# shijun18/H-DenseFormer

Hardware: AMD Instinct MI355X
Metric: train samples/sec on 4x128^3 volumes (higher is better)
Workload: dtype bf16

## Files before the change

h-denseformer_amd/csrc/transformer_chain.hip:

```cpp
#include <mutex>

#include "tf_tok.h"

namespace {

using namespace tftok;

constexpr int CT = 512;
constexpr int KVC = 128;
constexpr int KVP = 68;
constexpr int LDQ = 100;
constexpr int SYNC_LINE = 32;
constexpr int FR_KA = 0;
constexpr int FR_VA = 64;
constexpr int FR_QA = 128;
constexpr int FR_KB = 192;
constexpr int FR_QB = 232;
constexpr int FR_W = 288;
constexpr int XG_GA = 0;
constexpr int XG_GB = 64;
constexpr int XG_W = 128;
constexpr float LOG2E = 1.4426950408889634f, LN2 = 0.6931471805599453f;
constexpr int ATRIP = 16;
typedef float f2 __attribute__((ext_vector_type(2)));
// ... 186 lines not shown
}
__device__ __forceinline__ float4 ld16_sc1(__amdgpu_buffer_rsrc_t r, uint32_t byte_off) {
  return __builtin_bit_cast(float4, __builtin_amdgcn_raw_buffer_load_b128(r, byte_off, 0, 16));
}
__device__ __forceinline__ void chain_arrive(unsigned* cnt, bool storing = true) {
  if (storing) asm volatile("s_waitcnt vmcnt(0)" ::: "memory");
  __syncthreads();
  if (threadIdx.x == 0) __hip_atomic_fetch_add(cnt, 1u, __ATOMIC_RELAXED, __HIP_MEMORY_SCOPE_AGENT);
}
using ChainCtl = TfChainCtl;
__device__ __forceinline__ void chain_wait(unsigned* cnt, unsigned target, unsigned* tmo, const ChainCtl& c, bool& dead) {
  if (threadIdx.x == 0 && !dead) {
    const uint64_t t_start = __builtin_amdgcn_s_memrealtime();
    unsigned spins = 0;
    while (__hip_atomic_load(cnt, __ATOMIC_RELAXED, __HIP_MEMORY_SCOPE_AGENT) < target) {
      __builtin_amdgcn_s_sleep(2);
      if ((++spins & 31u) == 0u && __hip_atomic_load(tmo, __ATOMIC_RELAXED, __HIP_MEMORY_SCOPE_AGENT) != 0u) {
        dead = true;
        break;
      }
      if (__builtin_amdgcn_s_memrealtime() - t_start > (uint64_t)c.ticks) {
        __hip_atomic_store(tmo, 1u + blockIdx.x, __ATOMIC_RELAXED, __HIP_MEMORY_SCOPE_AGENT);
        if (c.host_flag) __hip_atomic_store(c.host_flag, 1u + blockIdx.x, __ATOMIC_RELAXED, __HIP_MEMORY_SCOPE_SYSTEM);
        dead = true;
        break;
      }
    }
  }
  __builtin_amdgcn_fence(__ATOMIC_ACQUIRE, "wavefront");
  __syncthreads();
}
__device__ __forceinline__ bool chain_any_dead(bool dead, unsigned* word) {
  __syncthreads();
  if (threadIdx.x == 0) *word = dead ? 1u : 0u;
  __syncthreads();
  return *word != 0u;
}

#ifdef CHAIN_DBG_STAMPS
#define CHAIN_STAMP(k)                                                                                   \
  do {                                                                                                   \
    if (threadIdx.x == 0)                                                                                \
      reinterpret_cast<uint64_t*>(a.sync + (1 << 18))[((size_t)blockIdx.x * 32 + L) * 16 + (k)] = __builtin_amdgcn_s_memrealtime(); \
  } while (0)
#define CHAIN_STAMPB(k)                                                                                  \
  do {                                                                                                   \
    if (threadIdx.x == 0)                                                                                \
      reinterpret_cast<uint64_t*>(a.sync + (1 << 18) + (1 << 17))[((size_t)blockIdx.x * 32 + (L + 1)) * 16 + (k)] = __builtin_amdgcn_s_memrealtime(); \
  } while (0)
#else
#define CHAIN_STAMP(k) ((void)0)
#define CHAIN_STAMPB(k) ((void)0)
#endif

struct ChainFwd {
  TfDims d;
  ChainW cw;
  const float* params;
  const float4* wpack;
  int dtype;
  float* F0;
  float* save;
  void* attnall;
  unsigned* sync;
  TfChainCtl ctl;
  float* frag;
  int nb, ntile, nseq;
  int64_t rows;
};

template <bool TRAIN>
__global__ __launch_bounds__(CT) void tf_chain_fwd_kernel(ChainFwd a) {
  HDF_CHAIN_PRIO();
  extern __shared__ __attribute__((aligned(16))) float sm[];
  const TfDims& d = a.d;
  const int DM = d.DM, DMF = d.DMF, ldF = DMF + 4, N = d.N, BN = d.B * N;
  float* s_F = sm;
  float* s_x = s_F + TT * ldF;
  float* s_h = s_x + TT * LD32;
  float* s_z = s_h + TT * LD32;
  float* s_red = s_z + TT * LD64;
  float* s_ob = s_red + 2 * 16 * 16;
  float* s_q = s_ob + TT * LD32;
  float* s_kv = s_q + TT * LDQ;
  const int tid = threadIdx.x, lane = tid & 63, wave8 = tid >> 6, wave = wave8 & 3, col = lane & 15, g = lane >> 4;
  const bool cw = tid < 256;
  const int seq = blockIdx.x % a.nseq, tile = blockIdx.x / a.nseq;
  const int m = seq / d.B, bsm = seq - m * d.B;
  const int n0 = tile * TT, nvalid = min(TT, N - n0);
  const int t0k = bsm * N + n0;
  const int64_t mo = (int64_t)m * d.mstride, rb = (int64_t)m * BN;
  const DropF dr{TRAIN ? 1 : 0, d.seed, d.thresh24, d.keep_scale};
  auto tok = [&](int row) { return t0k + min(row, nvalid - 1); };
  float* pm = const_cast<float*>(a.params);
  unsigned* cnt = a.sync + seq * SYNC_LINE;
  unsigned* tmo = a.sync + a.nseq * SYNC_LINE;
  bool dead = false;
  const int nl = a.nb * 4;
  const int cw_col = 16 * (wave & 1) + col, c4w = 16 * wave + col;

  WFrag<2> f_wo{}, f_w1{};
  WFrag<4> f_w2{};
  WFrag<11> f_w0{};
  WFrag<2> f_q0{}, f_q1{};
  float p_bout = 0.f, p_b1 = 0.f, p_b2 = 0.f, p_b0 = 0.f;
  LnP ln2{}, ln1{};
// ... 374 lines not shown
        const float inv = 1.f / l;
        const float4 o = make_float4(a01.x * inv, a01.y * inv, a23.x * inv, a23.y * inv);
        *reinterpret_cast<float4*>(s_ob + col * LD32 + head * 4) = o;
        const float lsv = __builtin_fmaf(mx, LN2, __logf(l));
        if (col < nvalid) {
          float* ob = sv + a.rows * 128;
          float* lse = sv + a.rows * 160;
          const int64_t R = rb + t0 + col;
          *reinterpret_cast<float4*>(ob + R * 32 + head * 4) = o;
          lse[R * 8 + head] = lsv;
        }
        if (a.frag)
          a.frag[(int64_t)nl * a.nseq * a.ntile * 8 * FR_W + (((int64_t)L * a.nseq + seq) * 8 + head) * (a.ntile * TT) + n0 + col] =
              col < nvalid ? -lsv * LOG2E : -INFINITY;
      }
      CHAIN_STAMP(7);
    }
  }
  if (chain_any_dead(dead, reinterpret_cast<unsigned*>(s_red))) {
    const float qnan = __builtin_nanf("");
    for (int i = tid; i < nvalid * DM; i += CT) {
      const int row = i / DM, c = i - row * DM;
      const int64_t ai = ((int64_t)bsm * N + n0 + row) * ((int64_t)d.M * DM) + (int64_t)m * DM + c;
      if (a.dtype == HDF_BF16)
        ST<bf16_t>::st(reinterpret_cast<bf16_t*>(a.attnall) + ai, qnan);
      else if (a.dtype == HDF_F16)
        ST<f16_t>::st(reinterpret_cast<f16_t*>(a.attnall) + ai, qnan);
      else
        reinterpret_cast<float*>(a.attnall)[ai] = qnan;
    }
  }
}

struct ChainBwd {
  TfDims d;
  ChainW cw;
  const float* params;
  float* grads;
  const float* F0;
  const float* save;
  float* dF;
  const void* d_attnall;
  const float4* wpack;
  float* tape;
  float* otape;
  float* xchg;
  const float* frag;
  unsigned* sync;
  TfChainCtl ctl;
  int nb, ntile, nseq, dtype;
  int64_t rows;
};

constexpr int QC = 64;
constexpr int QP = 84;
constexpr int XW = 40;

template <int LP>
struct ChainLp;
template <>
struct ChainLp<1> {
  static __device__ __forceinline__ uint16_t one(float v) { return f2bf(v); }
  static __device__ __forceinline__ u32x2 four(float a, float b, float c, float d) { return u32x2{pack_bf2(a, b), pack_bf2(c, d)}; }
  static __device__ __forceinline__ f32x4 mma(const u32x2& a, const u32x2& b, const f32x4& c) {
    return __builtin_amdgcn_mfma_f32_16x16x16bf16_1k(__builtin_bit_cast(s16x4, a), __builtin_bit_cast(s16x4, b), c, 0, 0, 0);
  }
};
typedef __attribute__((ext_vector_type(4))) _Float16 chain_f16x4;
template <>
struct ChainLp<2> {
  static __device__ __forceinline__ uint16_t one(float v) { return f2h(v); }
  static __device__ __forceinline__ u32x2 four(float a, float b, float c, float d) { return u32x2{pack_h2(a, b), pack_h2(c, d)}; }
  static __device__ __forceinline__ f32x4 mma(const u32x2& a, const u32x2& b, const f32x4& c) {
    return __builtin_amdgcn_mfma_f32_16x16x16f16(__builtin_bit_cast(chain_f16x4, a), __builtin_bit_cast(chain_f16x4, b), c, 0, 0, 0);
  }
};

__device__ __forceinline__ f32x4 chain_mfma4(float a, float b, const f32x4& c) {
  return __builtin_amdgcn_mfma_f32_16x16x4f32(a, b, c, 0, 0, 0);
}

template <bool TRAIN, int LP>
__global__ __launch_bounds__(CT) void tf_chain_bwd_kernel(ChainBwd a) {
  HDF_CHAIN_PRIO();
  extern __shared__ __attribute__((aligned(16))) float sm[];
  const TfDims& d = a.d;
  const int DM = d.DM, DMF = d.DMF, ldF = DMF + 4, ldD = DM + 4, N = d.N, BN = d.B * N;
  float* s_F = sm;
  float* s_dF = s_F + TT * ldF;
  float* s_do = s_dF + TT * ldF;
  float* s_dq = s_do + TT * ldD;
  float* s_a = s_dq + TT * 100;
  float* s_b = s_a + TT * LD32;
  float* s_c = s_b + TT * LD32;
  float* s_e = s_c + TT * LD32;
  float* s_dg = s_e + TT * LD32;
  float* s_gx = s_dg + TT * LD32;
  float* s_dO = s_gx + TT * LD32;
  float* s_f = s_dO + TT * LD32;
  float* s_dz = s_f + TT * LD64;
  float* s_red = s_dz + TT * LD64;
  float* s_dl = s_red + 2 * 16 * 16;
  float* s_at = s_dl + TT * 8;
  constexpr int AT_IMG = QC * QP, AT_T = 8 * QC, AT_U = 8 * 5 * QC / 2;
  constexpr int AT_BUF = AT_IMG + 2 * AT_T + 2 * AT_U;
  const int tid = threadIdx.x, lane = tid & 63, wave8 = tid >> 6, wave = wave8 & 3, col0 = lane & 15, g0 = lane >> 4;
  const bool cw = tid < 256;
  const int lrow0 = (tid >> 4) & 15, lc0 = (tid & 15) * 2;
  const int seq = blockIdx.x % a.nseq, tile = blockIdx.x / a.nseq;
  const int m = seq / d.B, bsm = seq - m * d.B;
  const int n0 = tile * TT, nvalid = min(TT, N - n0);
  const int t0k = bsm * N + n0;
  const int64_t mo = (int64_t)m * d.mstride, rb = (int64_t)m * BN;
  const int64_t trows = a.rows;
  const DropF dr{TRAIN ? 1 : 0, d.seed, d.thresh24, d.keep_scale};
  float* pm = const_cast<float*>(a.params);
  unsigned* cnt = a.sync + seq * SYNC_LINE;
  unsigned* tmo = a.sync + a.nseq * SYNC_LINE;
  bool dead = false;
  const int nl = a.nb * 4;
  float r_acc0 = 0.f, r_acc1 = 0.f;
  const int htid = tid - 256;

  for (int L = nl - 1; L >= -1; L--) {
    const bool PREB = L + 1 < nl, POSTB = L >= 0, OUTB = POSTB && (L & 3) == 3;
    const int Lq = L + 1, bq = Lq >> 2, lq = Lq & 3;
    const int bp = L >> 2, lp = L & 3, bo = bp;
    int t0 = t0k;
    asm volatile("" : "+s"(t0));
    int col = col0, g = g0, lrow = lrow0, lc = lc0;
    asm volatile("" : "+v"(col), "+v"(g), "+v"(lrow), "+v"(lc));
    auto tok = [&](int row) { return t0 + min(row, nvalid - 1); };
    auto tape_h = [&](float* tape, int col0, const float* sT, int lds_ld, int width) __attribute__((always_inline)) {
      const int w4 = width >> 2;
      float* seg = tape + trows * col0 + (rb + t0) * width;
      for (int i = htid; i < TT * w4; i += 256) {
        const int row = i / w4, c4 = (i - row * w4) * 4;
        if (row < nvalid) *reinterpret_cast<float4*>(seg + i * 4) = *reinterpret_cast<const float4*>(sT + row * lds_ld + c4);
      }
    };
    auto colsum_h = [&](float* gb, int width, const float* sv, int ld, int tbase) __attribute__((always_inline)) {
      const int c = htid - tbase;
      if (c >= 0 && c < width) {
        float acc = 0.f;
#pragma unroll
        for (int r = 0; r < TT; r++) acc += sv[r * ld + c];
        atomicAdd(gb + c, acc);
      }
    };
    const bool lok = lrow < nvalid;
    const int64_t lr = (rb + tok(lrow)) * 32 + lc;
    const int Kq = PREB ? DM + 32 * lq : 0;
    CFrag<12> c_q{};
    CFrag<8> c_w0[6]{};
    WFrag<2> f_w1{};
    CFrag<8> c_w2{}, c_w1{};
    CFrag<4> c_wo{};
    LnP ln1{}, ln2{};
    float p_b1 = 0.f, r_h[2][2] = {{0.f, 0.f}, {0.f, 0.f}}, r_ob[2] = {0.f, 0.f}, r_h0[2] = {0.f, 0.f};
    TfLayerP gq{}, gp{};
    if (PREB) {
      float* w0 = chain_w0(a.cw, pm, bq, lq) + mo;
      float* rest = w0 + 32 * Kq;
      float* gw0 = chain_w0(a.cw, a.grads, bq, lq) + mo;
      float* grest = gw0 + 32 * Kq;
      gq.b0 = grest + CO_B0, gq.ln1g = grest + CO_LN1G, gq.ln1b = grest + CO_LN1B;
      if (cw) {
        const float4* slot = a.wpack + ((int64_t)m * nl + Lq) * (CH_SLOT * 64);
        cpload(c_q, slot, CB_Q + 3 * wave);
#pragma unroll
        for (int j = 0; j < 6; j++) cpload(c_w0[j], slot, CB_W0 + 2 * min(wave + 4 * j, (Kq >> 4) - 1));
        ln1 = ln_load(rest + CO_LN1G, rest + CO_LN1B);
        const float* h0 = a.save + (int64_t)Lq * a.rows * 232;
        r_h0[0] = h0[lr], r_h0[1] = h0[lr + 1];
      }
    }
    if (POSTB) {
      float* w0 = chain_w0(a.cw, pm, bp, lp) + mo;
      float* rest = w0 + 32 * (DM + 32 * lp);
      float* grest = chain_w0(a.cw, a.grads, bp, lp) + mo + 32 * (DM + 32 * lp);
      gp.bout = grest + CO_BOUT, gp.ln2g = grest + CO_LN2G, gp.ln2b = grest + CO_LN2B, gp.b1 = grest + CO_B1, gp.b2 = grest + CO_B2;
      if (cw) {
        const float4* slot = a.wpack + ((int64_t)m * nl + L) * (CH_SLOT * 64);
        pload(f_w1, slot, CH_W1 + 2 * wave, 2);
// ... 133 lines not shown
        }
        {
          f32x4 acc = zero4();
          cmma_stream_p(acc, oslot, OB_B + 16 * wave, s_do, ldD, DM >> 2);
          const int c = 16 * wave + col;
#pragma unroll
          for (int r = 0; r < 4; r++) s_dz[(4 * g + r) * LD64 + c] = acc[r] * mk[r] * gelu_grad_f(zr[r]);
        }
      }
      __syncthreads();
      if (!cw) {
        tape_h(otape, 0, s_do, ldD, DM);
        tape_h(otape, DM, s_f, LD64, 64);
        tape_h(otape, DM + 64, s_dz, LD64, 64);
        for (int c0 = 0; c0 < DM; c0 += 128) colsum_h(go.bb + mo + c0, min(128, DM - c0), s_do + c0, ldD, 0);
        colsum_h(go.ba + mo, 64, s_dz, LD64, 128);
      } else {
        for (int nn = 16 * wave; nn < DMF; nn += 64) {
          f32x4 acc = zero4();
          cmma_stream_p(acc, oslot, OA_B + 4 * (nn >> 4), s_dz, LD64, 16);
          const int c = nn + col;
#pragma unroll
          for (int r = 0; r < 4; r++) {
            const int row = 4 * g + r;
            s_dF[row * ldF + c] = acc[r];
            if (c >= DMF - 32) s_dg[row * LD32 + c - (DMF - 32)] = row < nvalid ? acc[r] : 0.f;
          }
        }
      }
      __syncthreads();
    }

    CHAIN_STAMPB(3);
    {
      float* tape_p = a.tape + (int64_t)L * a.rows * TF_TAPE_W;
      const uint32_t site0 = hdf_site_id(m, bp, lp, 0);
      const int t = t0 + lrow;
      const bool ok = lok;
      float dcur0 = 0.f, dcur1 = 0.f;
      if (cw) dcur0 = s_dg[lrow * LD32 + lc], dcur1 = s_dg[lrow * LD32 + lc + 1];
      float dres0 = 0.f, dres1 = 0.f;
#pragma unroll
      for (int pass = 1; pass >= 0; pass--) {
        __syncthreads();
        float rs = 0.f;
        if (cw) {
          s_a[lrow * LD32 + lc] = r_h[pass][0];
          s_a[lrow * LD32 + lc + 1] = r_h[pass][1];
          rs = ln32_keep(s_a, s_b, s_c, ln2);
          s_dg[lrow * LD32 + lc] = ok ? dcur0 * dr.mask(site0 + 2 + 2 * pass, (uint32_t)t * 32 + lc) : 0.f;
          s_dg[lrow * LD32 + lc + 1] = ok ? dcur1 * dr.mask(site0 + 2 + 2 * pass, (uint32_t)t * 32 + lc + 1) : 0.f;
        }
        __syncthreads();
        if (pass == 1) CHAIN_STAMPB(9);
        if (cw) {
          f32x4 accz = zero4(), accd = zero4();
          wmma(accz, f_w1, s_b, LD32, 8, 0, 2);
          cmma(accd, c_w2, s_dg, LD32, 8, 0, 8);
          const int c = 16 * wave + col;
          const float b1 = p_b1;
#pragma unroll
          for (int r = 0; r < 4; r++) {
            const int row = 4 * g + r, tt = t0 + row;
            const float z = accz[r] + b1, mkv = dr.mask(site0 + 1 + 2 * pass, (uint32_t)tt * 64 + c);
            s_f[row * LD64 + c] = row < nvalid ? gelu_f(z) * mkv : 0.f;
            s_dz[row * LD64 + c] = row < nvalid ? accd[r] * mkv * gelu_grad_f(z) : 0.f;
          }
        }
        __syncthreads();
        if (pass == 1) CHAIN_STAMPB(10);
        f32x4 accu = zero4();
        if (!cw) {
          const int c0 = pass ? TF_T_P1 : TF_T_P0;
          tape_h(tape_p, c0, s_dg, LD32, 32);
          tape_h(tape_p, c0 + 32, s_f, LD64, 64);
          tape_h(tape_p, c0 + 96, s_dz, LD64, 64);
          tape_h(tape_p, c0 + 160, s_b, LD32, 32);
          colsum_h(gp.b2, 32, s_dg, LD32, 0);
          colsum_h(gp.b1, 64, s_dz, LD64, 64);
        } else {
          cmma(accu, c_w1, s_dz, LD64, 16, 8 * (wave >> 1), 8);
          if (wave >= 2) {
#pragma unroll
            for (int r = 0; r < 4; r++) s_red[((wave & 1) * 16 + 4 * g + r) * 16 + col] = accu[r];
          }
        }
        __syncthreads();
        if (pass == 1) CHAIN_STAMPB(11);
        if (cw && wave < 2) {
#pragma unroll
          for (int r = 0; r < 4; r++)
            s_e[(4 * g + r) * LD32 + 16 * wave + col] = accu[r] + s_red[(wave * 16 + 4 * g + r) * 16 + col];
        }
        __syncthreads();
        if (pass == 1) CHAIN_STAMPB(12);
        float dh0v = 0.f, dh1v = 0.f;
        if (cw) {
          ln32_bwd(s_e, s_c, s_gx, rs, ln2, dh0v, dh1v);
          dh0v = ok ? dh0v : 0.f, dh1v = ok ? dh1v : 0.f;
        }
        __syncthreads();
        if (pass == 1) CHAIN_STAMPB(13);
        if (!cw) {
          colsum_h(gp.ln2g, 32, s_gx, LD32, 0);
          colsum_h(gp.ln2b, 32, s_e, LD32, 64);
        }
        if (pass == 1) {
          dcur0 = dh0v, dcur1 = dh1v;
          dres0 = dh0v, dres1 = dh1v;
        } else {
          dres0 += dh0v, dres1 += dh1v;
        }
      }
      __syncthreads();
      if (cw) {
        s_dg[lrow * LD32 + lc] = ok ? dres0 * dr.mask(site0 + 0, (uint32_t)t * 32 + lc) : 0.f;
        s_dg[lrow * LD32 + lc + 1] = ok ? dres1 * dr.mask(site0 + 0, (uint32_t)t * 32 + lc + 1) : 0.f;
        s_b[lrow * LD32 + lc] = r_ob[0];
        s_b[lrow * LD32 + lc + 1] = r_ob[1];
        r_acc0 = dres0, r_acc1 = dres1;
      }
      __syncthreads();
      CHAIN_STAMPB(14);
      f32x4 acco = zero4();
      if (!cw) {
        tape_h(tape_p, TF_T_DGO, s_dg, LD32, 32);
        colsum_h(gp.bout, 32, s_dg, LD32, 0);
      } else {
        cmma(acco, c_wo, s_dg, LD32, 8, 4 * (wave >> 1), 4);
        if (wave >= 2) {
#pragma unroll
          for (int r = 0; r < 4; r++) s_red[((wave & 1) * 16 + 4 * g + r) * 16 + col] = acco[r];
        }
      }
      __syncthreads();
      if (cw && wave < 2) {
#pragma unroll
        for (int r = 0; r < 4; r++)
          s_dO[(4 * g + r) * LD32 + 16 * wave + col] = acco[r] + s_red[(wave * 16 + 4 * g + r) * 16 + col];
      }
      __syncthreads();
      CHAIN_STAMPB(15);
      if (tid < TT * 8) {
        const int row = tid >> 3, h = tid & 7;
        s_dl[row * 8 + h] = tf_dot4(*reinterpret_cast<const float4*>(s_dO + row * LD32 + 4 * h),
                                    *reinterpret_cast<const float4*>(s_b + row * LD32 + 4 * h));
      }
      __syncthreads();
    }

    CHAIN_STAMPB(4);
    const int par = L & 1;
    float* xbase = a.xchg + ((int64_t)par * a.rows + rb + (int64_t)bsm * N) * XW;
    const __amdgpu_buffer_rsrc_t rx = chain_rsrc(xbase);
    float* xgseq = a.xchg + ((int64_t)par * a.nseq + seq) * a.ntile * 8 * XG_W;
    if (LP) {
      constexpr int L1 = LP ? LP : 1;
      float* s_rec = s_f;
      {
        const int hd = wave8;
        float* rec = s_rec + hd * XG_W;
        const bool vrow = col < nvalid;
        rec[XG_GA + lane] = vrow ? s_dO[col * LD32 + hd * 4 + g] : 0.f;
        if (lane < 20) {
          const int c = lane >> 2, gg = lane & 3;
          float gv[4] = {0.f, 0.f, 0.f, 0.f};
          if (c < 4) {
#pragma unroll
            for (int e = 0; e < 4; e++) gv[e] = 4 * gg + e < nvalid ? s_dO[(4 * gg + e) * LD32 + hd * 4 + c] : 0.f;
          }
          reinterpret_cast<u32x2*>(rec + XG_GB)[lane] = ChainLp<L1>::four(gv[0], gv[1], gv[2], gv[3]);
        }
        if (lane < 16) rec[XG_GB + 40 + lane] = lane < nvalid ? -s_dl[lane * 8 + hd] : 0.f;
      }
      __syncthreads();
      if (tid < 8 * 26) {
        const int hd = tid / 26, pc = tid - hd * 26;
        const __amdgpu_buffer_rsrc_t rr = chain_rsrc(xgseq + (int64_t)tile * 8 * XG_W);
        st16_sc1(rr, (uint32_t)((hd * XG_W + 4 * pc) * 4), *reinterpret_cast<const float4*>(s_rec + hd * XG_W + 4 * pc));
      } else if (tid < 8 * 26 + 32) {
        const int i = tid - 8 * 26, hd = i >> 2, pc = i & 3;
        const __amdgpu_buffer_rsrc_t rr = chain_rsrc(a.xchg + (int64_t)2 * a.nseq * a.ntile * 8 * XG_W +
                                                     ((int64_t)par * a.nseq + seq) * 8 * (a.ntile * TT));
        st16_sc1(rr, (uint32_t)((hd * (a.ntile * TT) + n0 + 4 * pc) * 4),
                 *reinterpret_cast<const float4*>(s_rec + hd * XG_W + XG_GB + 40 + 4 * pc));
      }
    } else if (tid < TT * 10) {
      const int row = tid / 10, c4 = (tid - row * 10) * 4;
      if (row < nvalid) {
        const float4 v = c4 < 32 ? *reinterpret_cast<const float4*>(s_dO + row * LD32 + c4)
                                 : *reinterpret_cast<const float4*>(s_dl + row * 8 + (c4 - 32));
        st16_sc1(rx, (uint32_t)(((n0 + row) * XW + c4) * 4), v);
      }
    }
    const int head = __builtin_amdgcn_readfirstlane(wave8);
    const float* sv = a.save + (int64_t)L * a.rows * 232;
    const float* qkvL = sv + a.rows * 32 + (rb + (int64_t)bsm * N) * 96;
    const float* lseL = sv + a.rows * 160 + (rb + (int64_t)bsm * N) * 8;
    const int rown = n0 + min(col, nvalid - 1);
    const float own_q = qkvL[(int64_t)rown * 96 + head * 4 + g];
    const float own_k = qkvL[(int64_t)rown * 96 + 32 + head * 4 + g];
    const float own_v = qkvL[(int64_t)rown * 96 + 64 + head * 4 + g];
    const float own_lse = lseL[(int64_t)rown * 8 + head];
    constexpr int PD = 8, NLS = 4;
    const int NPq = attn_rows(N);
    const float* fr = nullptr;
    const int cb = min(col, 4) * 4 + g;
    float ka[PD], va[PD];
    u32x2 kb[PD];
    float4 r_ls[NLS];
    auto ldk = [&](int b, int i) __attribute__((always_inline)) {
      const float* r = fr + (int64_t)min(b, a.ntile - 1) * 8 * FR_W;
      ka[i] = r[FR_KA + lane], va[i] = r[FR_VA + lane];
      kb[i] = reinterpret_cast<const u32x2*>(r + FR_KB)[cb];
    };
    if constexpr (LP != 0) {
      fr = a.frag + ((int64_t)L * a.nseq + seq) * a.ntile * 8 * FR_W + (int64_t)head * FR_W;
      const float* lsrow = a.frag + (int64_t)nl * a.nseq * a.ntile * 8 * FR_W + (((int64_t)L * a.nseq + seq) * 8 + head) * NPq;
#pragma unroll
      for (int i = 0; i < PD; i++) ldk(i, i);
#pragma unroll
      for (int k = 0; k < NLS; k++) r_ls[k] = *reinterpret_cast<const float4*>(lsrow + min((k * 64 + lane) * 4, NPq - 4));
    }
    chain_arrive(cnt, cw);
    CHAIN_STAMPB(5);
    CHAIN_STAMPB(6);

    if constexpr (LP != 0) {
      const int NP = NPq, nblk = a.ntile;
      const float* xg = xgseq + (int64_t)head * XG_W;
      float* s_ls = s_at + head * 2 * NP;
      float* s_dlq = s_ls + NP;
      const __amdgpu_buffer_rsrc_t rdl = chain_rsrc(a.xchg + (int64_t)2 * a.nseq * a.ntile * 8 * XG_W +
                                                    (((int64_t)par * a.nseq + seq) * 8 + head) * NP);
      {
        const float delta = s_dl[col * 8 + head];
        const float ls = own_lse * LOG2E;
        const float bqv = own_q * (0.5f * LOG2E);
        const float bg = s_dO[col * LD32 + head * 4 + g];
        const f32x4 nl4 = {-ls, -ls, -ls, -ls}, nd4 = {-delta, -delta, -delta, -delta};
        f32x4 acc = {0.f, 0.f, 0.f, 0.f};
        auto step = [&](int i, int j0, auto masked) __attribute__((always_inline)) {
          const f32x4 cs = chain_mfma4(ka[i], bqv, nl4), ct = chain_mfma4(va[i], bg, nd4);
          float ds[4];
#pragma unroll
          for (int u = 0; u < 4; u++) {
            ds[u] = __builtin_amdgcn_exp2f(cs[u]) * ct[u];
            if (decltype(masked)::value) ds[u] = (j0 + 4 * g + u < N) ? ds[u] : 0.f;
          }
          acc = ChainLp<LP>::mma(ChainLp<LP>::four(ds[0], ds[1], ds[2], ds[3]), kb[i], acc);
        };
        const int nfullb = N / ATRIP;
        int bb = 0;
        for (; bb + PD <= nfullb; bb += PD) {
#pragma unroll
          for (int i = 0; i < PD; i++) {
            step(i, 0, std::false_type{});
            ldk(bb + i + PD, i);
          }
        }
        for (int i = 0; bb < nblk; bb++, i++) {
#pragma unroll
          for (int k = 0; k < PD; k++)
            if (k == i) {
              if ((bb + 1) * ATRIP <= N)
                step(k, 0, std::false_type{});
              else
                step(k, bb * ATRIP, std::true_type{});
            }
        }
#pragma unroll
        for (int r = 0; r < 4; r++)
          if (col < 4) s_dq[(4 * g + r) * 100 + head * 4 + col] = (4 * g + r < nvalid) ? 0.5f * acc[r] : 0.f;
      }
      chain_wait(cnt, (unsigned)(a.ntile * (nl - L)), tmo, a.ctl, dead);
      {
        float4 r_dl[NLS];
#pragma unroll
        for (int k = 0; k < NLS; k++) r_dl[k] = ld16_sc1(rdl, (uint32_t)(min((k * 64 + lane) * 4, NP - 4) * 4));
#pragma unroll
        for (int k = 0; k < NLS; k++) {
          const int i4 = (k * 64 + lane) * 4;
          if (i4 < NP) {
            *reinterpret_cast<float4*>(s_ls + i4) = r_ls[k];
            *reinterpret_cast<float4*>(s_dlq + i4) = r_dl[k];
          }
        }
      }
      CHAIN_STAMPB(7);
      {
        const float bk = own_k, bv = own_v;
        const float* tl = s_ls + 4 * g;
        const float* td = s_dlq + 4 * g;
        float qa[PD], ga[PD];
        u32x2 qb[PD], gb[PD];
        auto ld = [&](int b, int i) __attribute__((always_inline)) {
          const int bc = min(b, nblk - 1);
          const float* r = fr + (int64_t)bc * 8 * FR_W;
          const float* x = xg + (int64_t)bc * 8 * XG_W;
          qa[i] = r[FR_QA + lane];
          qb[i] = reinterpret_cast<const u32x2*>(r + FR_QB)[cb];
          ga[i] = __hip_atomic_load(x + XG_GA + lane, __ATOMIC_RELAXED, __HIP_MEMORY_SCOPE_AGENT);
          const unsigned long long w = __hip_atomic_load(reinterpret_cast<const unsigned long long*>(x + XG_GB) + cb,
                                                         __ATOMIC_RELAXED, __HIP_MEMORY_SCOPE_AGENT);
          gb[i] = u32x2{(uint32_t)w, (uint32_t)(w >> 32)};
        };
#pragma unroll
        for (int i = 0; i < PD; i++) ld(i, i);
        f32x4 dk = {0.f, 0.f, 0.f, 0.f}, dv = {0.f, 0.f, 0.f, 0.f};
        auto step = [&](int i, int b) __attribute__((always_inline)) {
          const f32x4 l4 = *reinterpret_cast<const f32x4*>(tl + b * ATRIP), d4 = *reinterpret_cast<const f32x4*>(td + b * ATRIP);
          const f32x4 cs = chain_mfma4(qa[i], bk, l4), ct = chain_mfma4(ga[i], bv, d4);
          const float p0 = __builtin_amdgcn_exp2f(cs[0]), p1 = __builtin_amdgcn_exp2f(cs[1]);
          const float p2 = __builtin_amdgcn_exp2f(cs[2]), p3 = __builtin_amdgcn_exp2f(cs[3]);
          dv = ChainLp<LP>::mma(ChainLp<LP>::four(p0, p1, p2, p3), gb[i], dv);
          dk = ChainLp<LP>::mma(ChainLp<LP>::four(p0 * ct[0], p1 * ct[1], p2 * ct[2], p3 * ct[3]), qb[i], dk);
        };
        int bb = 0;
        for (; bb + PD <= nblk; bb += PD) {
#pragma unroll
          for (int i = 0; i < PD; i++) {
            step(i, bb + i);
            ld(bb + i + PD, i);
          }
        }
        for (int i = 0; bb < nblk; bb++, i++) {
#pragma unroll
// ... 29 lines not shown
          const float z = c * QC + srow < N ? 1.f : 0.f;
          float* img = s_at + (c & 1) * AT_BUF;
          const float4 kk = make_float4(pk.x * z, pk.y * z, pk.z * z, pk.w * z);
          *reinterpret_cast<float4*>(img + srow * KVP + 4 * spart) = kk;
          *reinterpret_cast<float4*>(img + srow * KVP + 32 + 4 * spart) = make_float4(pv.x * z, pv.y * z, pv.z * z, pv.w * z);
          if (LP) {
            uint16_t* kt = reinterpret_cast<uint16_t*>(img + AT_IMG + 2 * AT_T) + spart * 5 * QC;
            constexpr int L1 = LP ? LP : 1;
            kt[0 * QC + srow] = ChainLp<L1>::one(kk.x), kt[1 * QC + srow] = ChainLp<L1>::one(kk.y);
            kt[2 * QC + srow] = ChainLp<L1>::one(kk.z), kt[3 * QC + srow] = ChainLp<L1>::one(kk.w);
            kt[4 * QC + srow] = 0;
          }
        };
        stage_load(0);
        stage_store(0);
        __syncthreads();
        f32x4 acc = {0.f, 0.f, 0.f, 0.f};
        f2 d01 = {0.f, 0.f}, d23 = {0.f, 0.f};
        const f32x4 nl4 = {-ls, -ls, -ls, -ls}, nd4 = {-delta, -delta, -delta, -delta}, z4 = {0.f, 0.f, 0.f, 0.f};
        for (int c = 0; c < nchunk; c++) {
          if (c + 1 < nchunk) stage_load(c + 1);
          const float* img = s_at + (c & 1) * AT_BUF;
          const uint16_t* kt = reinterpret_cast<const uint16_t*>(img + AT_IMG + 2 * AT_T) + head * 5 * QC + min(col, 4) * QC + 4 * g;
          const int jbase = c * QC, ntrip = min(QC, NP - jbase) / ATRIP;
          for (int k = 0; k < ntrip; k++) {
            const int jj = k * ATRIP, j0 = jbase + jj;
            const float ka = img[(jj + col) * KVP + head * 4 + g], va = img[(jj + col) * KVP + 32 + head * 4 + g];
            if (LP) {
              constexpr int L1 = LP ? LP : 1;
              const f32x4 cs = chain_mfma4(ka, bqv, nl4), ct = chain_mfma4(va, bg, nd4);
              const u32x2 kb = *reinterpret_cast<const u32x2*>(kt + jj);
              float ds[4];
#pragma unroll
              for (int u = 0; u < 4; u++) {
                ds[u] = __builtin_amdgcn_exp2f(cs[u]) * ct[u];
                if (j0 + ATRIP > N) ds[u] = (j0 + 4 * g + u < N) ? ds[u] : 0.f;
              }
              acc = ChainLp<L1>::mma(ChainLp<L1>::four(ds[0], ds[1], ds[2], ds[3]), kb, acc);
            } else {
              const f32x4 s4 = chain_mfma4(ka, bqv, z4), t4 = chain_mfma4(va, bg, z4);
#pragma unroll
              for (int u = 0; u < 4; u++) {
                const float4 kr = *reinterpret_cast<const float4*>(img + (jj + 4 * g + u) * KVP + head * 4);
                float pr = __builtin_amdgcn_exp2f(s4[u] - ls);
                if (j0 + ATRIP > N) pr = (j0 + 4 * g + u < N) ? pr : 0.f;
                const float dsv = pr * (t4[u] - delta);
                const f2 dd = {dsv, dsv};
                d01 = __builtin_elementwise_fma(dd, lo2(kr), d01);
                d23 = __builtin_elementwise_fma(dd, hi2(kr), d23);
              }
            }
          }
          if (c + 1 < nchunk) stage_store(c + 1);
          __syncthreads();
        }
        if (LP) {
#pragma unroll
          for (int r = 0; r < 4; r++)
            if (col < 4) s_dq[(4 * g + r) * 100 + head * 4 + col] = (4 * g + r < nvalid) ? 0.5f * acc[r] : 0.f;
        } else {
#pragma unroll
          for (int off = 16; off < 64; off <<= 1) {
            d01.x += __shfl_xor(d01.x, off, 64), d01.y += __shfl_xor(d01.y, off, 64);
            d23.x += __shfl_xor(d23.x, off, 64), d23.y += __shfl_xor(d23.y, off, 64);
          }
          if (g == 0)
            *reinterpret_cast<float4*>(s_dq + col * 100 + head * 4) =
                rvalid ? make_float4(0.5f * d01.x, 0.5f * d01.y, 0.5f * d23.x, 0.5f * d23.y) : make_float4(0.f, 0.f, 0.f, 0.f);
        }
      }
      chain_wait(cnt, (unsigned)(a.ntile * (nl - L)), tmo, a.ctl, dead);
      CHAIN_STAMPB(7);
      {
        const float bk = own_k, bv = own_v;
        float4 pq, pg, pl;
        auto stage_load = [&](int c) __attribute__((always_inline)) {
          const int j = min(c * QC + srow, N - 1);
          pq = *reinterpret_cast<const float4*>(qkvL + (int64_t)j * 96 + 4 * spart);
          pg = ld16_sc1(rx, (uint32_t)((j * XW + 4 * spart) * 4));
          if (spart < 2)
            pl = *reinterpret_cast<const float4*>(lseL + (int64_t)j * 8 + 4 * spart);
          else if (spart < 4)
            pl = ld16_sc1(rx, (uint32_t)((j * XW + 32 + 4 * (spart - 2)) * 4));
        };
        auto stage_store = [&](int c) __attribute__((always_inline)) {
          const bool real = c * QC + srow < N;
          const float z = real ? 1.f : 0.f, sc = real ? 0.5f * LOG2E : 0.f;
          float* img = s_at + (c & 1) * AT_BUF;
          float* tl = img + AT_IMG;
          float* td = tl + AT_T;
          *reinterpret_cast<float4*>(img + srow * QP + 4 * spart) = make_float4(pq.x * sc, pq.y * sc, pq.z * sc, pq.w * sc);
          if (LP) {
            constexpr int L1 = LP ? LP : 1;
            *reinterpret_cast<float4*>(img + srow * QP + 32 + 4 * spart) = make_float4(pg.x * z, pg.y * z, pg.z * z, pg.w * z);
            uint16_t* qt = reinterpret_cast<uint16_t*>(td + AT_T) + spart * 5 * QC;
            uint16_t* gt = qt + 8 * 5 * QC;
            qt[0 * QC + srow] = ChainLp<L1>::one(pq.x * z), qt[1 * QC + srow] = ChainLp<L1>::one(pq.y * z);
            qt[2 * QC + srow] = ChainLp<L1>::one(pq.z * z), qt[3 * QC + srow] = ChainLp<L1>::one(pq.w * z);
            qt[4 * QC + srow] = 0;
            gt[0 * QC + srow] = ChainLp<L1>::one(pg.x * z), gt[1 * QC + srow] = ChainLp<L1>::one(pg.y * z);
            gt[2 * QC + srow] = ChainLp<L1>::one(pg.z * z), gt[3 * QC + srow] = ChainLp<L1>::one(pg.w * z);
            gt[4 * QC + srow] = 0;
            if (spart < 2) {
              const int h4 = 4 * spart;
              tl[(h4 + 0) * QC + srow] = real ? -pl.x * LOG2E : -INFINITY, tl[(h4 + 1) * QC + srow] = real ? -pl.y * LOG2E : -INFINITY;
              tl[(h4 + 2) * QC + srow] = real ? -pl.z * LOG2E : -INFINITY, tl[(h4 + 3) * QC + srow] = real ? -pl.w * LOG2E : -INFINITY;
            } else if (spart < 4) {
              const int h4 = 4 * (spart - 2);
              td[(h4 + 0) * QC + srow] = -z * pl.x, td[(h4 + 1) * QC + srow] = -z * pl.y;
              td[(h4 + 2) * QC + srow] = -z * pl.z, td[(h4 + 3) * QC + srow] = -z * pl.w;
            }
          } else {
            *reinterpret_cast<float4*>(img + srow * QP + 32 + 4 * spart) =
                make_float4(real ? pg.x : 0.f, real ? pg.y : 0.f, real ? pg.z : 0.f, real ? pg.w : 0.f);
            if (spart < 2) {
              const int h4 = 4 * spart;
              tl[(h4 + 0) * QC + srow] = real ? pl.x * LOG2E : INFINITY, tl[(h4 + 1) * QC + srow] = real ? pl.y * LOG2E : INFINITY;
              tl[(h4 + 2) * QC + srow] = real ? pl.z * LOG2E : INFINITY, tl[(h4 + 3) * QC + srow] = real ? pl.w * LOG2E : INFINITY;
            } else if (spart < 4) {
              const int h4 = 4 * (spart - 2);
              td[(h4 + 0) * QC + srow] = real ? pl.x : 0.f, td[(h4 + 1) * QC + srow] = real ? pl.y : 0.f;
              td[(h4 + 2) * QC + srow] = real ? pl.z : 0.f, td[(h4 + 3) * QC + srow] = real ? pl.w : 0.f;
            }
// ... 26 lines not shown
              const float p2 = __builtin_amdgcn_exp2f(cs[2]), p3 = __builtin_amdgcn_exp2f(cs[3]);
              dv = ChainLp<L1>::mma(ChainLp<L1>::four(p0, p1, p2, p3), gb, dv);
              dk = ChainLp<L1>::mma(ChainLp<L1>::four(p0 * ct[0], p1 * ct[1], p2 * ct[2], p3 * ct[3]), qb, dk);
            } else {
              const f32x4 cs = chain_mfma4(qa, bk, z4), ct = chain_mfma4(ga, bv, z4);
#pragma unroll
              for (int u = 0; u < 4; u++) {
                const float4 qr = *reinterpret_cast<const float4*>(img + (ii + 4 * g + u) * QP + head * 4);
                const float4 gr = *reinterpret_cast<const float4*>(img + (ii + 4 * g + u) * QP + 32 + head * 4);
                const float pr = __builtin_amdgcn_exp2f(cs[u] - l4[u]);
                const f2 pp = {pr, pr};
                dv01 = __builtin_elementwise_fma(pp, lo2(gr), dv01);
                dv23 = __builtin_elementwise_fma(pp, hi2(gr), dv23);
                const float dsv = pr * (ct[u] - d4[u]);
                const f2 dd = {dsv, dsv};
                dk01 = __builtin_elementwise_fma(dd, lo2(qr), dk01);
                dk23 = __builtin_elementwise_fma(dd, hi2(qr), dk23);
              }
            }
          }
          if (c + 1 < nchunk) stage_store(c + 1);
          __syncthreads();
        }
        if (LP) {
#pragma unroll
          for (int r = 0; r < 4; r++) {
            if (col < 4) {
              const bool ok = 4 * g + r < nvalid;
              s_dq[(4 * g + r) * 100 + 32 + head * 4 + col] = ok ? 0.5f * dk[r] : 0.f;
              s_dq[(4 * g + r) * 100 + 64 + head * 4 + col] = ok ? dv[r] : 0.f;
            }
          }
        } else {
#pragma unroll
          for (int off = 16; off < 64; off <<= 1) {
            dk01.x += __shfl_xor(dk01.x, off, 64), dk01.y += __shfl_xor(dk01.y, off, 64);
            dk23.x += __shfl_xor(dk23.x, off, 64), dk23.y += __shfl_xor(dk23.y, off, 64);
            dv01.x += __shfl_xor(dv01.x, off, 64), dv01.y += __shfl_xor(dv01.y, off, 64);
            dv23.x += __shfl_xor(dv23.x, off, 64), dv23.y += __shfl_xor(dv23.y, off, 64);
          }
          if (g == 0) {
            const float un = 1.f / LOG2E;
            const float4 z = make_float4(0.f, 0.f, 0.f, 0.f);
            *reinterpret_cast<float4*>(s_dq + col * 100 + 32 + head * 4) =
                rvalid ? make_float4(dk01.x * un, dk01.y * un, dk23.x * un, dk23.y * un) : z;
            *reinterpret_cast<float4*>(s_dq + col * 100 + 64 + head * 4) =
                rvalid ? make_float4(dv01.x, dv01.y, dv23.x, dv23.y) : z;
          }
        }
      }
    }
    CHAIN_STAMPB(8);
  }
  if (chain_any_dead(dead, reinterpret_cast<unsigned*>(s_red))) {
    const float qnan = __builtin_nanf("");
    for (int i = tid; i < nvalid * DM; i += CT) {
      const int row = i / DM, c = i - row * DM;
      a.dF[(rb + t0k + row) * DMF + c] = qnan;
    }
  }
}

size_t chain_bwd_lds(const TfDims& d, int dtype) {
  const size_t tiles = (size_t)2 * TT * (d.DMF + 4) + TT * (d.DM + 4) + TT * 100 + 7 * TT * LD32 + 2 * TT * LD64 + 2 * 16 * 16 + TT * 8;
  const size_t att = dtype == HDF_F32 ? (size_t)2 * (QC * QP + 2 * 8 * QC + 2 * (8 * 5 * QC / 2)) : (size_t)2 * 8 * attn_rows(d.N);
  return (tiles + att) * sizeof(float);
}

size_t chain_fwd_lds(const TfDims& d) {
  return (size_t)(TT * (d.DMF + 4) + 2 * TT * LD32 + TT * LD64 + 2 * 16 * 16 + TT * LD32 + TT * LDQ + 2 * KVC * KVP) *
         sizeof(float);
}

template <typename Kern>
int chain_allow_lds(Kern kern, size_t bytes) {
  if (bytes <= 64 * 1024) return HDF_OK;
  hipError_t e = hipFuncSetAttribute(reinterpret_cast<const void*>(kern), hipFuncAttributeMaxDynamicSharedMemorySize,
                                     (int)LDS_LIMIT_F);
  if (e != hipSuccess) {
    hdf_set_error("hipFuncSetAttribute(MaxDynamicSharedMemorySize) failed: %s", hipGetErrorString(e));
    return HDF_ERR_HIP;
  }
  return HDF_OK;
}

}

static bool chain_digest(const TfChainP& cp, int DM, ChainW& w) {
  static const int rel[13] = {0, CO_B0, CO_LN1G, CO_LN1B, CO_WQKV, CO_WOUT, CO_BOUT, CO_LN2G, CO_LN2B, CO_W1, CO_B1, CO_W2, CO_B2};
  for (int l = 0; l < 4; l++) {
    w.l0[l] = cp.loff[l][0];
    for (int k = 1; k < 13; k++)
      if (cp.loff[l][k] != cp.loff[l][0] + 32 * (DM + 32 * l) + rel[k]) return false;
  }
  for (int k = 0; k < 4; k++) w.ooff[k] = cp.ooff[k];
  w.blk0 = cp.blk0, w.blk_stride = cp.blk_stride;
  return true;
}

size_t tf_chain_sync_bytes(const TfDims& d) { return (size_t)(d.M * d.B + 1) * SYNC_LINE * sizeof(unsigned); }
bool tf_chain_supported(const TfDims& d);
size_t tf_chain_frag_bytes(const TfDims& d, int nb) {
  const size_t nt = ceil_div(d.N, TT);
  return (size_t)nb * 4 * d.M * d.B * (nt * 8 * FR_W + 8 * nt * TT) * sizeof(float);
}
bool tf_chain_backward_supported(const TfDims& d, int dtype) {
  return tf_chain_supported(d) && chain_bwd_lds(d, dtype) <= LDS_LIMIT_F &&
         (dtype == HDF_F32 || ((size_t)2 * d.M * d.B * ceil_div(d.N, TT) * (8 * XG_W + 8 * TT) <= (size_t)d.M * d.B * d.N * 160 &&
                               attn_rows(d.N) <= 1024));
}
size_t tf_chain_wpack_bytes(const TfDims& d, int nb) {
// ... 130 lines not shown
```

Baseline: 187.0.

## Defer backward chain arrive into attention loop and rematerialize per-layer kernel args

Moves the cross-block chain_arrive signal from before the attention dQ loop to inside it: after a configurable block in the low-precision path, and in place of the first chunk's barrier in the f32 path. Peers waiting on the counter therefore start later, but the arriving block has more of its own work in flight. Separately, per-layer index and pointer setup is re-derived each iteration from the kernarg segment instead of being held live across the loop, aiming to cut register pressure. Also adds debug-stamp variants. The later arrive risks longer waits by dependent blocks, and the arrive-replaces-barrier substitution relies on chain_arrive providing the same synchronization.

```diff
diff --git a/h-denseformer_amd/csrc/transformer_chain.hip b/h-denseformer_amd/csrc/transformer_chain.hip
--- a/h-denseformer_amd/csrc/transformer_chain.hip
+++ b/h-denseformer_amd/csrc/transformer_chain.hip
@@ -262,6 +262,13 @@
 #define CHAIN_STAMP(k) ((void)0)
 #define CHAIN_STAMPB(k) ((void)0)
 #endif
+#if defined(CHAIN_DBG_STAMPS) && (CHAIN_DBG_STAMPS + 0) == 2
+#define CHAIN_STAMPB_POST(k) ((void)0)
+#define CHAIN_STAMPB_PUB(k) CHAIN_STAMPB(k)
+#else
+#define CHAIN_STAMPB_POST(k) CHAIN_STAMPB(k)
+#define CHAIN_STAMPB_PUB(k) ((void)0)
+#endif
 
 struct ChainFwd {
   TfDims d;
@@ -742,6 +749,9 @@
   int64_t rows;
 };
 
+#ifndef CHAIN_BWD_ARRIVE_BLK
+#define CHAIN_BWD_ARRIVE_BLK 0
+#endif
 constexpr int QC = 64;
 constexpr int QP = 84;
 constexpr int XW = 40;
@@ -770,56 +780,62 @@
   return __builtin_amdgcn_mfma_f32_16x16x4f32(a, b, c, 0, 0, 0);
 }
 
+template <typename A>
+__device__ __forceinline__ const A& chain_args() {
+  auto p = __builtin_amdgcn_kernarg_segment_ptr();
+  asm volatile("" : "+s"(p));
+  return *(const A*)p;
+}
+
 template <bool TRAIN, int LP>
 __global__ __launch_bounds__(CT) void tf_chain_bwd_kernel(ChainBwd a) {
   HDF_CHAIN_PRIO();
   extern __shared__ __attribute__((aligned(16))) float sm[];
-  const TfDims& d = a.d;
-  const int DM = d.DM, DMF = d.DMF, ldF = DMF + 4, ldD = DM + 4, N = d.N, BN = d.B * N;
-  float* s_F = sm;
-  float* s_dF = s_F + TT * ldF;
-  float* s_do = s_dF + TT * ldF;
-  float* s_dq = s_do + TT * ldD;
-  float* s_a = s_dq + TT * 100;
-  float* s_b = s_a + TT * LD32;
-  float* s_c = s_b + TT * LD32;
-  float* s_e = s_c + TT * LD32;
-  float* s_dg = s_e + TT * LD32;
-  float* s_gx = s_dg + TT * LD32;
-  float* s_dO = s_gx + TT * LD32;
-  float* s_f = s_dO + TT * LD32;
-  float* s_dz = s_f + TT * LD64;
-  float* s_red = s_dz + TT * LD64;
-  float* s_dl = s_red + 2 * 16 * 16;
-  float* s_at = s_dl + TT * 8;
   constexpr int AT_IMG = QC * QP, AT_T = 8 * QC, AT_U = 8 * 5 * QC / 2;
   constexpr int AT_BUF = AT_IMG + 2 * AT_T + 2 * AT_U;
-  const int tid = threadIdx.x, lane = tid & 63, wave8 = tid >> 6, wave = wave8 & 3, col0 = lane & 15, g0 = lane >> 4;
-  const bool cw = tid < 256;
-  const int lrow0 = (tid >> 4) & 15, lc0 = (tid & 15) * 2;
-  const int seq = blockIdx.x % a.nseq, tile = blockIdx.x / a.nseq;
-  const int m = seq / d.B, bsm = seq - m * d.B;
-  const int n0 = tile * TT, nvalid = min(TT, N - n0);
-  const int t0k = bsm * N + n0;
-  const int64_t mo = (int64_t)m * d.mstride, rb = (int64_t)m * BN;
-  const int64_t trows = a.rows;
-  const DropF dr{TRAIN ? 1 : 0, d.seed, d.thresh24, d.keep_scale};
-  float* pm = const_cast<float*>(a.params);
-  unsigned* cnt = a.sync + seq * SYNC_LINE;
-  unsigned* tmo = a.sync + a.nseq * SYNC_LINE;
+  const int seq0 = blockIdx.x % a.nseq, tile0 = blockIdx.x / a.nseq;
+  const int m0 = seq0 / a.d.B, bsm0 = seq0 - m0 * a.d.B;
   bool dead = false;
   const int nl = a.nb * 4;
   float r_acc0 = 0.f, r_acc1 = 0.f;
-  const int htid = tid - 256;
 
   for (int L = nl - 1; L >= -1; L--) {
+    const ChainBwd& a = chain_args<ChainBwd>();
+    const TfDims& d = a.d;
+    int seq = seq0, tile = tile0, m = m0, bsm = bsm0, tid = threadIdx.x;
+    asm volatile("" : "+s"(seq), "+s"(tile), "+s"(m), "+s"(bsm), "+v"(tid));
+    const int DM = d.DM, DMF = d.DMF, ldF = DMF + 4, ldD = DM + 4, N = d.N, BN = d.B * N;
+    float* s_F = sm;
+    float* s_dF = s_F + TT * ldF;
+    float* s_do = s_dF + TT * ldF;
+    float* s_dq = s_do + TT * ldD;
+    float* s_a = s_dq + TT * 100;
+    float* s_b = s_a + TT * LD32;
+    float* s_c = s_b + TT * LD32;
+    float* s_e = s_c + TT * LD32;
+    float* s_dg = s_e + TT * LD32;
+    float* s_gx = s_dg + TT * LD32;
+    float* s_dO = s_gx + TT * LD32;
+    float* s_f = s_dO + TT * LD32;
+    float* s_dz = s_f + TT * LD64;
+    float* s_red = s_dz + TT * LD64;
+    float* s_dl = s_red + 2 * 16 * 16;
+    float* s_at = s_dl + TT * 8;
+    const int lane = tid & 63, wave8 = tid >> 6, wave = wave8 & 3, col = lane & 15, g = lane >> 4;
+    const bool cw = tid < 256;
+    const int lrow = (tid >> 4) & 15, lc = (tid & 15) * 2;
+    const int htid = tid - 256;
+    const int n0 = tile * TT, nvalid = min(TT, N - n0);
+    const int t0 = bsm * N + n0;
+    const int64_t mo = (int64_t)m * d.mstride, rb = (int64_t)m * BN;
+    const int64_t trows = a.rows;
+    const DropF dr{TRAIN ? 1 : 0, d.seed, d.thresh24, d.keep_scale};
+    float* pm = const_cast<float*>(a.params);
+    unsigned* cnt = a.sync + seq * SYNC_LINE;
+    unsigned* tmo = a.sync + a.nseq * SYNC_LINE;
     const bool PREB = L + 1 < nl, POSTB = L >= 0, OUTB = POSTB && (L & 3) == 3;
     const int Lq = L + 1, bq = Lq >> 2, lq = Lq & 3;
     const int bp = L >> 2, lp = L & 3, bo = bp;
-    int t0 = t0k;
-    asm volatile("" : "+s"(t0));
-    int col = col0, g = g0, lrow = lrow0, lc = lc0;
-    asm volatile("" : "+v"(col), "+v"(g), "+v"(lrow), "+v"(lc));
     auto tok = [&](int row) { return t0 + min(row, nvalid - 1); };
     auto tape_h = [&](float* tape, int col0, const float* sT, int lds_ld, int width) __attribute__((always_inline)) {
       const int w4 = width >> 2;
@@ -1059,7 +1075,7 @@
           s_dg[lrow * LD32 + lc + 1] = ok ? dcur1 * dr.mask(site0 + 2 + 2 * pass, (uint32_t)t * 32 + lc + 1) : 0.f;
         }
         __syncthreads();
-        if (pass == 1) CHAIN_STAMPB(9);
+        if (pass == 1) CHAIN_STAMPB_POST(9);
         if (cw) {
           f32x4 accz = zero4(), accd = zero4();
           wmma(accz, f_w1, s_b, LD32, 8, 0, 2);
@@ -1075,7 +1091,7 @@
           }
         }
         __syncthreads();
-        if (pass == 1) CHAIN_STAMPB(10);
+        if (pass == 1) CHAIN_STAMPB_POST(10);
         f32x4 accu = zero4();
         if (!cw) {
           const int c0 = pass ? TF_T_P1 : TF_T_P0;
@@ -1093,21 +1109,21 @@
           }
         }
         __syncthreads();
-        if (pass == 1) CHAIN_STAMPB(11);
+        if (pass == 1) CHAIN_STAMPB_POST(11);
         if (cw && wave < 2) {
 #pragma unroll
           for (int r = 0; r < 4; r++)
             s_e[(4 * g + r) * LD32 + 16 * wave + col] = accu[r] + s_red[(wave * 16 + 4 * g + r) * 16 + col];
         }
         __syncthreads();
-        if (pass == 1) CHAIN_STAMPB(12);
+        if (pass == 1) CHAIN_STAMPB_POST(12);
         float dh0v = 0.f, dh1v = 0.f;
         if (cw) {
           ln32_bwd(s_e, s_c, s_gx, rs, ln2, dh0v, dh1v);
           dh0v = ok ? dh0v : 0.f, dh1v = ok ? dh1v : 0.f;
         }
         __syncthreads();
-        if (pass == 1) CHAIN_STAMPB(13);
+        if (pass == 1) CHAIN_STAMPB_POST(13);
         if (!cw) {
           colsum_h(gp.ln2g, 32, s_gx, LD32, 0);
           colsum_h(gp.ln2b, 32, s_e, LD32, 64);
@@ -1181,6 +1197,7 @@
         if (lane < 16) rec[XG_GB + 40 + lane] = lane < nvalid ? -s_dl[lane * 8 + hd] : 0.f;
       }
       __syncthreads();
+      CHAIN_STAMPB_PUB(9);
       if (tid < 8 * 26) {
         const int hd = tid / 26, pc = tid - hd * 26;
         const __amdgpu_buffer_rsrc_t rr = chain_rsrc(xgseq + (int64_t)tile * 8 * XG_W);
@@ -1200,6 +1217,7 @@
         st16_sc1(rx, (uint32_t)(((n0 + row) * XW + c4) * 4), v);
       }
     }
+    CHAIN_STAMPB_PUB(10);
     const int head = __builtin_amdgcn_readfirstlane(wave8);
     const float* sv = a.save + (int64_t)L * a.rows * 232;
     const float* qkvL = sv + a.rows * 32 + (rb + (int64_t)bsm * N) * 96;
@@ -1210,6 +1228,7 @@
     const float own_v = qkvL[(int64_t)rown * 96 + 64 + head * 4 + g];
     const float own_lse = lseL[(int64_t)rown * 8 + head];
     constexpr int PD = 8, NLS = 4;
+    constexpr int ARRIVE_BLK = CHAIN_BWD_ARRIVE_BLK;
     const int NPq = attn_rows(N);
     const float* fr = nullptr;
     const int cb = min(col, 4) * 4 + g;
@@ -1229,9 +1248,7 @@
 #pragma unroll
       for (int k = 0; k < NLS; k++) r_ls[k] = *reinterpret_cast<const float4*>(lsrow + min((k * 64 + lane) * 4, NPq - 4));
     }
-    chain_arrive(cnt, cw);
     CHAIN_STAMPB(5);
-    CHAIN_STAMPB(6);
 
     if constexpr (LP != 0) {
       const int NP = NPq, nblk = a.ntile;
@@ -1265,6 +1282,11 @@
             step(i, 0, std::false_type{});
             ldk(bb + i + PD, i);
           }
+          if (bb == ARRIVE_BLK) {
+            CHAIN_STAMPB_PUB(11);
+            chain_arrive(cnt, cw);
+            CHAIN_STAMPB_PUB(12);
+          }
         }
         for (int i = 0; bb < nblk; bb++, i++) {
 #pragma unroll
@@ -1279,7 +1301,9 @@
 #pragma unroll
         for (int r = 0; r < 4; r++)
           if (col < 4) s_dq[(4 * g + r) * 100 + head * 4 + col] = (4 * g + r < nvalid) ? 0.5f * acc[r] : 0.f;
-      }
+        if (ARRIVE_BLK + PD > nfullb) chain_arrive(cnt, cw);
+      }
+      CHAIN_STAMPB(6);
       chain_wait(cnt, (unsigned)(a.ntile * (nl - L)), tmo, a.ctl, dead);
       {
         float4 r_dl[NLS];
@@ -1415,7 +1439,10 @@
             }
           }
           if (c + 1 < nchunk) stage_store(c + 1);
-          __syncthreads();
+          if (c == 0)
+            chain_arrive(cnt, cw);
+          else
+            __syncthreads();
         }
         if (LP) {
 #pragma unroll
@@ -1432,6 +1459,7 @@
                 rvalid ? make_float4(0.5f * d01.x, 0.5f * d01.y, 0.5f * d23.x, 0.5f * d23.y) : make_float4(0.f, 0.f, 0.f, 0.f);
         }
       }
+      CHAIN_STAMPB(6);
       chain_wait(cnt, (unsigned)(a.ntile * (nl - L)), tmo, a.ctl, dead);
       CHAIN_STAMPB(7);
       {
@@ -1564,11 +1592,15 @@
     }
     CHAIN_STAMPB(8);
   }
-  if (chain_any_dead(dead, reinterpret_cast<unsigned*>(s_red))) {
-    const float qnan = __builtin_nanf("");
-    for (int i = tid; i < nvalid * DM; i += CT) {
-      const int row = i / DM, c = i - row * DM;
-      a.dF[(rb + t0k + row) * DMF + c] = qnan;
+  {
+    const int DM = a.d.DM, DMF = a.d.DMF, N = a.d.N, tid = threadIdx.x;
+    const int nvalid = min(TT, N - tile0 * TT);
+    if (chain_any_dead(dead, reinterpret_cast<unsigned*>(sm))) {
+      const float qnan = __builtin_nanf("");
+      for (int i = tid; i < nvalid * DM; i += CT) {
+        const int row = i / DM, c = i - row * DM;
+        a.dF[((int64_t)m0 * a.d.B * N + bsm0 * N + tile0 * TT + row) * DMF + c] = qnan;
+      }
     }
   }
 }
```

After: 188.5 (median of 6 runs). No clear change (+0.8%).
